# COMP6248-Reproducability-Challenge/selfsupervised-denoising

Hardware: AMD Instinct MI355X
Metric: training patches/sec (64x64 gauss25 SSDN) (higher is better)
Workload: dtype f16

## Files before the change

### include/ssdn_hip.h

```cpp
#ifndef SSDN_HIP_H
#define SSDN_HIP_H

#include <stdint.h>

#ifdef __cplusplus
extern "C" {
#endif
#if defined(__GNUC__) || defined(__clang__)
#pragma GCC visibility push(default)
#endif

#define SSDN_ABI_VERSION 19
#define SSDN_MAX_TAPS 9

typedef struct ssdn_view {
    void* p;
    int32_t cs;
    int32_t co;
} ssdn_view;

enum ssdn_op_type {
    SSDN_OP_PACK_INPUT = 1,
    SSDN_OP_CONV = 2,
    SSDN_OP_POOL_FWD = 3,
// ... 362 lines not shown
int ssdn_run_ops(const ssdn_op* ops, int n, void* stream);

int ssdn_stream_order(void* first, void* then);

int ssdn_conv_lds_bytes(const ssdn_conv_args* a);
int ssdn_wgrad_lds_bytes(const ssdn_wgrad_args* a);
int ssdn_wgrad_mega_ok(const ssdn_wgrad_args* a);
int ssdn_wgrad_variant(const ssdn_wgrad_args* a, int32_t* out9);

int ssdn_struct_size(int op_type);
int ssdn_abi_version(void);
const char* ssdn_last_error(void);
int ssdn_device_cus(void);

#define SSDN_PROF_CONV_MT3 0
#define SSDN_PROF_CONV_MT2 1
#define SSDN_PROF_CONV_MT1 2
#define SSDN_PROF_WGRAD 3
#define SSDN_PROF_GEMM 4
#define SSDN_PROF_CDMA_MT3 5
#define SSDN_PROF_CDMA_MT21 6
#define SSDN_PROF_WGRAD_SIDE 7
#define SSDN_PROF_KINDS 8
int ssdn_profile_enable(int kind, int max_launches);
int ssdn_profile_set_stride(int kind, int stride);
int ssdn_profile_read(int kind, double* total_ms, long long* launches, double* flops, double* bytes);

int ssdn_conv_set_mode(int mode);
int ssdn_conv_fuses_pool(const ssdn_conv_args* a);
int ssdn_conv_fuses_upsum(const ssdn_conv_args* a);
int ssdn_conv_fuses_unrot(const ssdn_conv_args* a);
int ssdn_conv_fuses_urot(const ssdn_conv_args* a);
int ssdn_conv_signs(const ssdn_conv_args* a);

int ssdn_chain_len(const ssdn_op* ops, int n);
int ssdn_conv_set_chain(int on);

int ssdn_wgrad_mergeable(const ssdn_wgrad_args* a);

#define SSDN_PLAN_REPACK 0
#define SSDN_PLAN_FORWARD 1
#define SSDN_PLAN_BACKWARD 2
#define SSDN_PLAN_OPTIMISER 3
#define SSDN_PLAN_PHASES 4
typedef struct ssdn_plan ssdn_plan;
int ssdn_plan_load(const void* blob, int64_t nbytes, ssdn_plan** out);
void ssdn_plan_destroy(ssdn_plan* plan);
int64_t ssdn_plan_arena_bytes(const ssdn_plan* plan);
const char* ssdn_plan_meta(const ssdn_plan* plan);
int ssdn_plan_bind(ssdn_plan* plan, void* arena);
int ssdn_plan_tensor(const ssdn_plan* plan, const char* name, void** ptr, int64_t* bytes);
int ssdn_plan_run(ssdn_plan* plan, int phase, void* stream);
int ssdn_plan_set_lr(ssdn_plan* plan, float lr, int step, float gscale);
int ssdn_net_forward(ssdn_plan* plan, void* stream);
int ssdn_train_step(ssdn_plan* plan, float lr, int step, void* stream);

void ssdn_debug_set_trace(void* device_buffer);
void* ssdn_debug_get_trace(void);

int ssdn_probe_mfma(const void* a_frag, const void* b_frag, float* d_out, void* stream);
int ssdn_probe_tr16(const void* lds_image, int image_bytes, const int32_t* lane_addr, void* out, void* stream);

#if defined(__GNUC__) || defined(__clang__)
#pragma GCC visibility pop
#endif
#ifdef __cplusplus
// ... 4 lines not shown
```

### selfsupervised-denoising_amd/csrc/api.hip

```cpp
#include "common.h"
#include <cstdarg>
#include <cstdio>
#include <cstdlib>

static thread_local char g_err[512] = "";
thread_local hipEvent_t g_ssdn_stop_event = nullptr;
thread_local bool g_ssdn_stop_used = false;
thread_local hipEvent_t g_ssdn_prof_start = nullptr, g_ssdn_prof_stop = nullptr;
thread_local bool g_ssdn_prof_used = false;

int ssdn_set_error(const char* fmt, ...) {
    va_list ap;
    va_start(ap, fmt);
    vsnprintf(g_err, sizeof(g_err), fmt, ap);
    va_end(ap);
    return -1;
}

#include <vector>
struct ProfSlot {
    bool on = false;
    std::vector<hipEvent_t> ev;
    size_t used = 0;
    double flops = 0.0, bytes = 0.0;
// ... 107 lines not shown
    if (stride < 1) return ssdn_set_error("profile: stride must be >= 1");
    g_prof[kind].stride = stride;
    return 0;
}

int ssdn_profile_read(int kind, double* total_ms, long long* launches, double* flops, double* bytes) {
    if (kind < 0 || kind >= SSDN_PROF_KINDS) return ssdn_set_error("profile: bad kernel kind %d", kind);
    ProfSlot& p = g_prof[kind];
    double ms = 0.0;
    for (size_t i = 0; i + 1 < p.used; i += 2) {
        if (hipEventSynchronize(p.ev[i + 1]) != hipSuccess) return ssdn_set_error("profile: hipEventSynchronize failed");
        float t = 0.f;
        if (hipEventElapsedTime(&t, p.ev[i], p.ev[i + 1]) != hipSuccess) return ssdn_set_error("profile: hipEventElapsedTime failed");
        ms += t;
    }
    *total_ms = ms;
    *launches = (long long)(p.used / 2);
    *flops = p.flops;
    *bytes = p.bytes;
    p.used = 0;
    p.flops = p.bytes = 0.0;
    return 0;
}

int ssdn_conv_lds_bytes(const ssdn_conv_args* a) { return conv_lds_bytes(a); }
int ssdn_wgrad_lds_bytes(const ssdn_wgrad_args* a) { return wgrad_lds_bytes(a); }
int ssdn_wgrad_mergeable(const ssdn_wgrad_args* a) { return a && wgrad_mergeable(a) ? 1 : 0; }
int ssdn_wgrad_mega_ok(const ssdn_wgrad_args* a) { return wgrad_mega_ok(a); }
int ssdn_conv_fuses_pool(const ssdn_conv_args* a) { return a && conv_fuses_pool(a) ? 1 : 0; }
int ssdn_conv_fuses_upsum(const ssdn_conv_args* a) { return a && conv_fuses_upsum(a) ? 1 : 0; }
int ssdn_conv_fuses_unrot(const ssdn_conv_args* a) { return a && conv_fuses_unrot(a) ? 1 : 0; }
int ssdn_conv_fuses_urot(const ssdn_conv_args* a) { return a && conv_fuses_urot(a) ? 1 : 0; }
int ssdn_conv_signs(const ssdn_conv_args* a) { return a && conv_signs(a) ? 1 : 0; }

#define SSDN_NEVENTS 256
#define SSDN_NLANES 4
#define SSDN_MAX_DEVICES 16
struct LaneSet {
    hipStream_t side[SSDN_NLANES] = {nullptr, nullptr, nullptr, nullptr};
    hipEvent_t ev[SSDN_NEVENTS];
    int ev_next = 0;
    bool ready = false;
};
static LaneSet g_lanesets[SSDN_MAX_DEVICES];
static LaneSet* lanes_get() {
    int dev = 0;
    if (hipGetDevice(&dev) != hipSuccess || dev < 0 || dev >= SSDN_MAX_DEVICES) { ssdn_set_error("lanes: bad current device"); return nullptr; }
    LaneSet& L = g_lanesets[dev];
    if (L.ready) return &L;
    for (int l = 1; l < SSDN_NLANES; ++l)
        if (hipStreamCreateWithFlags(&L.side[l], hipStreamNonBlocking) != hipSuccess) { ssdn_set_error("lanes: hipStreamCreate failed"); return nullptr; }
    for (int i = 0; i < SSDN_NEVENTS; ++i)
        if (hipEventCreateWithFlags(&L.ev[i], hipEventDisableTiming) != hipSuccess) { ssdn_set_error("lanes: hipEventCreate failed"); return nullptr; }
    L.ready = true;
    return &L;
}
static const unsigned g_lane_deps[SSDN_NLANES] = {0u, 1u << 0, (1u << 0) | (1u << 1) | (1u << 3), 1u << 0};

int ssdn_stream_order(void* first, void* then) {
    LaneSet* LS = lanes_get();
    if (!LS) return -1;
    hipEvent_t e = LS->ev[LS->ev_next++ % SSDN_NEVENTS];
    SSDN_CHECK_HIP(hipEventRecord(e, (hipStream_t)first));
    SSDN_CHECK_HIP(hipStreamWaitEvent((hipStream_t)then, e, 0));
    return 0;
}
// ... 265 lines not shown
```

### selfsupervised-denoising_amd/csrc/common.h

```cpp
#pragma once
#include <hip/hip_runtime.h>
#include <hip/hip_ext.h>
#include <stdint.h>
#include "../../include/ssdn_hip.h"
#include <cstdlib>

#if defined(SSDN_TUNING)
static inline const char* ssdn_tuning_env(const char* name) { return std::getenv(name); }
#else
static inline const char* ssdn_tuning_env(const char*) { return nullptr; }
#endif

typedef _Float16 h16;
typedef _Float16 half8 __attribute__((ext_vector_type(8)));
typedef _Float16 half4 __attribute__((ext_vector_type(4)));
typedef _Float16 half2v __attribute__((ext_vector_type(2)));
typedef __bf16 bf16x8 __attribute__((ext_vector_type(8)));
typedef unsigned short u16x8 __attribute__((ext_vector_type(8)));
typedef unsigned short u16x4 __attribute__((ext_vector_type(4)));
typedef float f32x16 __attribute__((ext_vector_type(16)));
typedef float f32x4 __attribute__((ext_vector_type(4)));

#define LRELU_SLOPE 0.1f

// ... 105 lines not shown
int launch_spatial_mean(const ssdn_spatial_mean_args* a, hipStream_t s);
int launch_mse(const ssdn_mse_args* a, int masked, hipStream_t s);
int launch_head_vjp(const ssdn_head_vjp_args* a, hipStream_t s);
int launch_head_vjp_impulse(const ssdn_head_vjp_args* a, hipStream_t s);
int launch_head_posterior(const ssdn_head_posterior_args* a, hipStream_t s);
int launch_ssim(const ssdn_ssim_args* a, hipStream_t s);
int launch_calibration(const ssdn_calibration_args* a, hipStream_t s);
int launch_mse_vjp(const ssdn_mse_vjp_args* a, hipStream_t s);
int launch_adam(const ssdn_adam_args* a, hipStream_t s);
#define ADAM_PACK_MAX 24
int adam_pack_fusable(const ssdn_adam_args* a, const ssdn_wpack_args* const* items, int n);
int launch_adam_pack(const ssdn_adam_args* a, const ssdn_wpack_args* const* items, int n, hipStream_t s);
int tail_fused_ok(const ssdn_wreduce_args* const* wr, int nw, const ssdn_adam_args* a, const ssdn_wpack_args* const* wp, int np);
int launch_tail_fused(const ssdn_wreduce_args* const* wr, int nw, const ssdn_adam_args* a, const ssdn_wpack_args* const* wp, int np, hipStream_t s);
int launch_metrics(const ssdn_metrics_args* a, hipStream_t s);
int launch_accum(const ssdn_accum_args* a, hipStream_t s);
int launch_noise(const ssdn_noise_args* a, hipStream_t s);
int launch_input_grad(const ssdn_input_grad_args* a, hipStream_t s);
int conv_lds_bytes(const ssdn_conv_args* a);
int conv_validate(const ssdn_conv_args* a);
int chain_len(const ssdn_op* ops, int n, bool any_lane);
int launch_chain(const ssdn_op* ops, int n, bool any_lane, hipStream_t s);
bool chain_merging_on();
bool conv_dma_eligible(const ssdn_conv_args* a, bool any_size);
int conv_dma_lds_bytes(int mt);
bool conv_signs(const ssdn_conv_args* a);
bool gemm_dma_signs(const ssdn_conv_args* a);
bool conv_dma_signs(const ssdn_conv_args* a);
bool conv_fuses_urot(const ssdn_conv_args* a);
bool conv_fuses_unrot(const ssdn_conv_args* a);
bool conv_fuses_upsum(const ssdn_conv_args* a);
bool conv_fuses_pool(const ssdn_conv_args* a);
int launch_conv_dma(const ssdn_conv_args* a, hipStream_t s);
bool conv_thin_eligible(const ssdn_conv_args* a);
bool conv_thin_fuses_pack(const ssdn_pack_input_args* pk, const ssdn_conv_args* a);
int launch_conv_thin(const ssdn_conv_args* a, const ssdn_pack_input_args* pk, hipStream_t s);
bool conv_pack_fusable(const ssdn_pack_input_args* pk, const ssdn_conv_args* a);
bool gradpack_dgrad_fusable(const ssdn_grad_pack_args* gp, const ssdn_conv_args* a);
int launch_gradpack_dgrad(const ssdn_grad_pack_args* gp, const ssdn_conv_args* a, hipStream_t s);
bool conv_gradpack_fusable(const ssdn_grad_pack_args* gp, const ssdn_conv_args* a);
bool gemm_dma_eligible(const ssdn_conv_args* a);
int gemm_dma_lds_bytes(const ssdn_conv_args* a);
int launch_gemm_dma(const ssdn_conv_args* a, hipStream_t s);
bool gemm_dma_fuses_next(const ssdn_conv_args* a, const ssdn_conv_args* b);
int launch_gemm_dma_with_next(const ssdn_conv_args* a, const ssdn_conv_args* b, hipStream_t s);
bool conv_pair_fusable(const ssdn_conv_args* a, const ssdn_conv_args* b);
extern "C" int ssdn_device_cus(void);
int wgrad_lds_bytes(const ssdn_wgrad_args* a);
```

### selfsupervised-denoising_amd/csrc/conv_mfma.hip

```cpp
#include "common.h"
#ifdef SSDN_TUNING
#define CV_ABL(xx, bit) (((xx).ablate & (bit)) != 0)
#define CV_TUNING 1
#else
#define CV_ABL(xx, bit) false
#define CV_TUNING 0
#endif
#include <cstdlib>


struct ConvGeom {
    int TW, TH, TN, HH, HW, padT, padB, padL, padR;
    int PSTR, WSTR, NP;
    int tiles_x, tiles_y, groups_n;
};

static __host__ __device__ inline ConvGeom conv_geom(int ltw, int lth, int ltn, int ntaps, const int* dy, const int* dx,
                                                     int N, int H, int W, int kc) {
    ConvGeom g;
    g.TW = 1 << ltw; g.TH = 1 << lth; g.TN = 1 << ltn;
    int mny = 0, mxy = 0, mnx = 0, mxx = 0;
    for (int t = 0; t < ntaps; ++t) {
        mny = dy[t] < mny ? dy[t] : mny; mxy = dy[t] > mxy ? dy[t] : mxy;
        mnx = dx[t] < mnx ? dx[t] : mnx; mxx = dx[t] > mxx ? dx[t] : mxx;
// ... 631 lines not shown
                    }
                    if (has_mask) {
                        v0 *= lrelu_grad(f16_lo(mb[w]));
                        v1 *= lrelu_grad(f16_hi(mb[w]));
                    }
                    o[w] = BF ? pack_bf16x2(v0, v1) : pack_f16x2(v0, v1);
                }
            }
            __builtin_amdgcn_raw_buffer_store_b128(o, rd[u], go[u], 0, 0);
        }
    }
    stamp();
}

static bool conv_uses_mt1(const ssdn_conv_args* a, const ConvGeom& g) {
    static int mt1_tiles = -1;
    if (mt1_tiles < 0) {
        const char* e = ssdn_tuning_env("SSDN_CONV_MT1_TILES");
        mt1_tiles = e ? atoi(e) : ssdn_device_cus();
        if (mt1_tiles <= 0) mt1_tiles = 256;
    }
    return !a->dst32 && g.tiles_x * g.tiles_y * g.groups_n <= mt1_tiles && a->Mpad >= 64;
}

static int g_conv_mode = [] { const char* e = ssdn_tuning_env("SSDN_CONV_DMA"); return e ? atoi(e) : 1; }();
extern "C" int ssdn_conv_set_mode(int mode) {
    if (mode < 0 || mode > 2) return ssdn_set_error("conv mode must be 0, 1 or 2");
    g_conv_mode = mode;
    return 0;
}
static bool conv_use_dma(const ssdn_conv_args* a) { return g_conv_mode > 0 && !a->pool.p && conv_dma_eligible(a, g_conv_mode == 2); }
static bool conv_use_gemm(const ssdn_conv_args* a) { return g_conv_mode > 0 && gemm_dma_eligible(a); }
static bool conv_use_thin(const ssdn_conv_args* a) { return g_conv_mode > 0 && conv_thin_eligible(a); }
bool conv_gradpack_fusable(const ssdn_grad_pack_args* gp, const ssdn_conv_args* a) {
    return !conv_validate(a) && !conv_use_gemm(a) && !conv_use_thin(a) && !conv_use_dma(a) && gradpack_dgrad_fusable(gp, a);
}
bool conv_pair_fusable(const ssdn_conv_args* a, const ssdn_conv_args* b) {
    return !conv_validate(a) && !conv_validate(b) && conv_use_gemm(a) && gemm_dma_fuses_next(a, b);
}
bool conv_pack_fusable(const ssdn_pack_input_args* pk, const ssdn_conv_args* a) {
    return !conv_validate(a) && !conv_use_gemm(a) && conv_use_thin(a) && conv_thin_fuses_pack(pk, a);
}

int conv_validate(const ssdn_conv_args* a) {
    if (a->ntaps < 1 || a->ntaps > SSDN_MAX_TAPS) return ssdn_set_error("conv: ntaps out of range");
    if (a->ltw + a->lth + a->ltn > 9 || a->ltw < 0 || a->lth < 0 || a->ltn < 0) return ssdn_set_error("conv: tile must have <= 512 pixels");
    if (a->Ktot != a->c0 + a->c1 || (a->Ktot & 15)) return ssdn_set_error("conv: Ktot must equal c0+c1 and be a multiple of 16");
    if ((a->c0 & 7) || (a->c1 & 7)) return ssdn_set_error("conv: source channel counts must be multiples of 8");
    if (a->kc < 16 || (a->kc & 15) || a->Ktot % a->kc || (a->kc > 64 && a->kc != 96)) return ssdn_set_error("conv: kc must be 16, 32, 48, 64 or 96 and divide Ktot");
    if ((a->Mpad & 31) || a->M > a->Mpad) return ssdn_set_error("conv: Mpad must be a multiple of 32 and >= M");
    if (!a->dst32 && ((a->M & 7) || (a->dst.co & 7) || (a->dst.cs & 7))) return ssdn_set_error("conv: 16-bit output needs M, dst.co, dst.cs %% 8 == 0");
    if (a->add.p && ((a->add.co & 7) || (a->add.cs & 7))) return ssdn_set_error("conv: add view must be 16-byte aligned");
    if (a->mask.p && ((a->mask.co & 7) || (a->mask.cs & 7))) return ssdn_set_error("conv: mask view must be 16-byte aligned");
    if (a->up0 && ((a->H | a->W) & 1)) return ssdn_set_error("conv: upsampled source needs even H, W");
    if (a->c1 > 0 && !a->src1.p) return ssdn_set_error("conv: src1 missing");
    if (a->bf16 && a->dst32) return ssdn_set_error("conv: fp32 output is only implemented for the fp16 (forward) role");
    int csmax = a->src0.cs > a->src1.cs ? a->src0.cs : a->src1.cs;
    if ((long long)a->N * a->H * a->W * csmax >= (1ll << 31)) return ssdn_set_error("conv: tensor too large for 32-bit element offsets");
    return 0;
}

static size_t conv_lds(const ssdn_conv_args* a, const ConvGeom& g, int mt) {
    size_t main_b = (conv_async(*a, a->kc) ? 2 * (size_t)g.NP * a->kc * 2 : (size_t)g.NP * g.PSTR) + 2 * (size_t)mt * 32 * g.WSTR;
    if (conv_allw(*a, g, mt, a->kc) && !conv_async(*a, a->kc)) main_b = (size_t)g.NP * g.PSTR + 9 * (size_t)32 * g.WSTR;
    size_t epi_b = a->dst32 ? 0 : (size_t)(g.TN * g.TH * g.TW) * (mt * 64 + 16) + mt * 32 * 4;
    return main_b > epi_b ? main_b : epi_b;
}

int conv_lds_bytes(const ssdn_conv_args* a) {
    if (conv_validate(a)) return -1;
    if (conv_use_gemm(a)) return gemm_dma_lds_bytes(a);
    if (conv_use_thin(a)) return 32 * 1024;
    if (conv_use_dma(a)) return conv_dma_lds_bytes(a->Mpad >= 96 ? 3 : a->Mpad / 32);
    ConvGeom g = conv_geom(a->ltw, a->lth, a->ltn, a->ntaps, a->dy, a->dx, a->N, a->H, a->W, a->kc);
    int mt = a->Mpad / 32;
    if (mt > 3) mt = 3;
    if (conv_uses_mt1(a, g)) mt = 1;
    else if (a->kc == 96) { ssdn_set_error("conv: kc = 96 is only built for layers that run as 32-channel blocks (<= 1 tile per CU)"); return -1; }
    return (int)conv_lds(a, g, mt);
}

static bool conv_flat_ok(const ssdn_conv_args* a, const ConvGeom& g, int ks, int threads) {
    static const bool no_flat = ssdn_tuning_env("SSDN_CONV_NO_FLAT") != nullptr;
    const int m_last = a->M - (a->Mpad - 32);
    return !no_flat && threads == 256 && ks <= 4 && g.TW == a->W && g.TH == a->H && g.TN * g.TH * g.TW == 256 && a->N % g.TN == 0 &&
           (m_last == 32 || m_last == 16 || m_last == 8) && (!a->up0 || !((a->H | a->W) & 1));
}

template <int MT, bool BF, int KS, int CONV_THREADS>
static int conv_launch_mt(const ssdn_conv_args* a, const ConvGeom& g, ConvAux x, int nblk_y, hipStream_t s) {
    size_t lds = conv_lds(a, g, MT);
    if (lds > 160 * 1024) return ssdn_set_error("conv: tiling needs %zu B of LDS (> 160 KiB)", lds);
    static bool attr_set_dev[SSDN_MAX_DEVICES_ATTR] = {};
    bool& attr_set = attr_set_dev[ssdn_current_device_slot()];
    if (!attr_set) {
        SSDN_CHECK_HIP(hipFuncSetAttribute((const void*)k_conv<MT, BF, KS, CONV_THREADS>, hipFuncAttributeMaxDynamicSharedMemorySize, 160 * 1024));
        attr_set = true;
    }
    int grid = g.tiles_x * g.tiles_y * g.groups_n;
    int m_real = a->M - x.m_base;
    m_real = m_real < 0 ? 0 : (m_real > nblk_y * MT * 32 ? nblk_y * MT * 32 : m_real);
    double px = (double)a->N * a->H * a->W;
    const int kreal = a->kreal > 0 ? a->kreal : a->Ktot;
    double flops = 2.0 * px * m_real * kreal * a->ntaps;
    double bytes = px * (a->c0 * 2.0 / (a->up0 ? 4.0 : 1.0) + a->c1 * 2.0) + px * m_real * (a->dst32 ? 4.0 : 2.0);
    prof_begin(3 - MT, s);
// ... 45 lines not shown
bool conv_signs(const ssdn_conv_args* a) {
    if (!(a->sign_out || a->mask_sign || a->upsum_mask_sign) || conv_validate(a)) return false;
    if (conv_use_gemm(a)) return !a->upsum_mask_sign && gemm_dma_signs(a);
    if (conv_use_thin(a)) return a->sign_out && !a->mask_sign && !a->upsum_mask_sign;
    return conv_use_dma(a) && conv_dma_signs(a);
}
bool conv_fuses_urot(const ssdn_conv_args* a) {
    return a->urot.p && !conv_validate(a) && !conv_use_gemm(a) && !conv_use_thin(a) && conv_use_dma(a);
}
bool conv_fuses_unrot(const ssdn_conv_args* a) {
    ssdn_conv_args q = *a;
    if (!q.unrot.p) { q.unrot = q.dst; q.unrot_mask = q.dst; }
    return !conv_validate(&q) && conv_use_gemm(&q);
}
bool conv_fuses_upsum(const ssdn_conv_args* a) {
    if (conv_validate(a) || !a->bf16 || a->dst32 || a->mask.p || a->add.p || (a->H & 1) || (a->W & 1)) return false;
    if ((a->upsum_c & 7) || a->upsum_c > a->M || a->upsum_c <= 0) return false;
    if (conv_use_gemm(a)) return false;
    if (conv_use_dma(a)) return a->upsum_c % 96 == 0;
    return conv_flat_path(a);
}

int launch_conv(const ssdn_conv_args* a, hipStream_t s) {
    int rc = conv_validate(a);
    if (rc) return rc;
    if ((a->sign_out || a->mask_sign || a->upsum_mask_sign) && !conv_signs(a)) return ssdn_set_error("conv: sign bytes requested for a launch that cannot write / read them (ssdn_conv_signs)");
    if (a->urot.p && !conv_fuses_urot(a)) return ssdn_set_error("conv: fused UNROT_FWD requested for a launch that cannot fuse it (ssdn_conv_fuses_urot)");
    if (a->unrot.p && !conv_fuses_unrot(a)) return ssdn_set_error("conv: fused UNROT_BWD requested for a launch that cannot fuse it (ssdn_conv_fuses_unrot)");
    if (a->upsum.p && !conv_fuses_upsum(a)) return ssdn_set_error("conv: fused upsum requested for a launch that cannot fuse it (ssdn_conv_fuses_upsum)");
    if (a->pool.p && !conv_fuses_pool(a)) return ssdn_set_error("conv: fused max-pool requested for a launch that cannot fuse it (ssdn_conv_fuses_pool)");
    if (conv_use_gemm(a)) return launch_gemm_dma(a, s);
    if (conv_use_thin(a)) return launch_conv_thin(a, nullptr, s);
    if (conv_use_dma(a)) return launch_conv_dma(a, s);
    ConvGeom g = conv_geom(a->ltw, a->lth, a->ltn, a->ntaps, a->dy, a->dx, a->N, a->H, a->W, a->kc);
    ConvAux x;
    x.mg_hw = magic_of(g.HW);
    x.mg_hh = magic_of(g.HH);
    x.mg_ntaps = magic_of(a->ntaps);
    x.m_base = 0;
    {
        static const int env_ablate = [] { const char* e = ssdn_tuning_env("SSDN_CONV_ABLATE"); return e ? atoi(e) : 0; }();
        static const int env_desync = [] { const char* e = ssdn_tuning_env("SSDN_CONV_DESYNC"); return e ? atoi(e) : 0; }();
        x.ablate = env_ablate;
        x.trace = g_conv_trace;
        x.desync = env_desync;
    }
    int full = a->Mpad / 96, rem = (a->Mpad % 96) / 32;
    const bool bf = a->bf16 != 0;
    if (conv_uses_mt1(a, g)) {
        rc = bf ? conv_launch_ks<1, true>(a, g, x, a->Mpad / 32, s) : conv_launch_ks<1, false>(a, g, x, a->Mpad / 32, s);
        if (rc) return rc;
        SSDN_CHECK_HIP(hipGetLastError());
        return 0;
    }
    if (full) {
        rc = bf ? conv_launch_ks<3, true>(a, g, x, full, s) : conv_launch_ks<3, false>(a, g, x, full, s);
        if (rc) return rc;
    }
    x.m_base = full * 96;
    if (rem == 2) rc = bf ? conv_launch_ks<2, true>(a, g, x, 1, s) : conv_launch_ks<2, false>(a, g, x, 1, s);
    else if (rem == 1) rc = bf ? conv_launch_ks<1, true>(a, g, x, 1, s) : conv_launch_ks<1, false>(a, g, x, 1, s);
    if (rc) return rc;
    SSDN_CHECK_HIP(hipGetLastError());
    return 0;
}
```

### selfsupervised-denoising_amd/ssdn/hip/lib.py

```python
from __future__ import annotations

import ctypes as C
import os

_HERE = os.path.dirname(os.path.abspath(__file__))
LIB_PATH = os.environ.get("SSDN_HIP_LIB") or os.path.join(_HERE, "libssdn_hip.so")
MAX_TAPS = 9

OP = dict(pack_input=1, conv=2, pool_fwd=3, pool_bwd=4, upsum_bwd=5, unrot_fwd=6, unrot_bwd=7, wgrad=8, wreduce=9,
          wpack=10, grad_pack=11, head_ssdn=12, head_final=13, spatial_mean=14, mse=15, mask_mse=16, adam=17,
          metrics=18, zero=19, event_record=20, noise=21, input_grad=22, head_vjp=23,
          mse_vjp=24, accum=25, head_posterior=26, ssim=27, calibration=28)

i32, f32, vp = C.c_int32, C.c_float, C.c_void_p


class View(C.Structure):
    _fields_ = [("p", vp), ("cs", i32), ("co", i32)]


class OpRec(C.Structure):
    _fields_ = [("type", i32), ("lane", i32), ("args", vp)]


# ... 126 lines not shown
SSIM_WIN, SSIM_TILE_H, SSIM_TILE_W = 11, 16, 32


def ssim_scratch_bytes(B: int, Cn: int, H: int, W: int) -> int:
    tiles = lambda n, t: (n - (SSIM_WIN - 1) + t - 1) // t
    return 8 * B * Cn * tiles(H, SSIM_TILE_H) * tiles(W, SSIM_TILE_W)


class CalibrationArgs(C.Structure):
    _fields_ = [("mean", vp), ("cov", vp), ("ref", vp), ("ext", vp), ("B", i32), ("C", i32), ("H", i32), ("W", i32), ("stats", vp),
                ("hist", vp), ("zmap", vp), ("scratch", vp), ("scratch_bytes", C.c_int64)]


CALIB_BLOCK, CALIB_NSTATS, CALIB_HIST_BINS = 256, 12, 34


def calib_scratch_bytes(B: int, Cn: int, H: int, W: int) -> int:
    return 8 * CALIB_NSTATS * B * ((H * W + CALIB_BLOCK - 1) // CALIB_BLOCK)


ARG_TYPES = dict(pack_input=PackInputArgs, conv=ConvArgs, pool_fwd=PoolArgs, pool_bwd=PoolArgs, upsum_bwd=UpsumArgs,
                 unrot_fwd=UnrotArgs, unrot_bwd=UnrotArgs, wgrad=WgradArgs, wreduce=WreduceArgs, wpack=WpackArgs,
                 grad_pack=GradPackArgs, head_ssdn=HeadArgs, head_final=HeadFinalArgs, spatial_mean=SpatialMeanArgs,
                 mse=MseArgs, mask_mse=MseArgs, adam=AdamArgs, metrics=MetricsArgs, zero=ZeroArgs, event_record=EventArgs, noise=NoiseArgs,
                 input_grad=InputGradArgs, head_vjp=HeadVjpArgs, mse_vjp=MseVjpArgs, accum=AccumArgs,
                 head_posterior=HeadPosteriorArgs, ssim=SsimArgs, calibration=CalibrationArgs)

ABI_VERSION = 19

SYMBOLS = ["ssdn_run_ops", "ssdn_stream_order", "ssdn_conv_lds_bytes", "ssdn_wgrad_lds_bytes", "ssdn_abi_version", "ssdn_last_error",
           "ssdn_device_cus", "ssdn_probe_mfma", "ssdn_probe_tr16", "ssdn_struct_size", "ssdn_profile_enable",
           "ssdn_profile_read", "ssdn_profile_set_stride", "ssdn_debug_set_trace", "ssdn_debug_get_trace", "ssdn_conv_set_mode",
           "ssdn_wgrad_mergeable", "ssdn_conv_fuses_pool", "ssdn_conv_fuses_upsum", "ssdn_conv_fuses_unrot", "ssdn_conv_fuses_urot", "ssdn_conv_signs", "ssdn_chain_len",
           "ssdn_conv_set_chain", "ssdn_wgrad_mega_ok", "ssdn_wgrad_variant",
           "ssdn_plan_load", "ssdn_plan_destroy", "ssdn_plan_arena_bytes", "ssdn_plan_meta", "ssdn_plan_bind", "ssdn_plan_tensor", "ssdn_plan_run",
           "ssdn_plan_set_lr", "ssdn_net_forward", "ssdn_train_step"]
PLAN_PHASES = dict(repack=0, forward=1, backward=2, optimiser=3)
PROF = dict(conv_mt3=0, conv_mt2=1, conv_mt1=2, wgrad=3, gemm=4, cdma_mt3=5, cdma_mt21=6, wgrad_side=7)

def pointer_fields(st, base: int = 0):
    out = []
    for name, ty in st._fields_:
        off = base + getattr(st, name).offset
        if ty is vp:
            out.append(off)
        elif isinstance(ty, type) and issubclass(ty, C.Structure):
            out += pointer_fields(ty, off)
    return out


_lib = None


class SsdnHipError(RuntimeError):
    pass


def load() -> C.CDLL:
    global _lib
    if _lib is not None:
        return _lib
    if not os.path.exists(LIB_PATH):
        raise SsdnHipError("libssdn_hip.so not found at %s -- build it with `python -c 'import __graft_entry__ as g; g.build()'` "
                           "(the ssdn hot path has no CPU fallback)" % LIB_PATH)
    lib = C.CDLL(LIB_PATH)
    lib.ssdn_run_ops.argtypes = [C.POINTER(OpRec), C.c_int, vp]
    lib.ssdn_run_ops.restype = C.c_int
# ... 3 lines not shown
    lib.ssdn_conv_lds_bytes.argtypes = [C.POINTER(ConvArgs)]
    lib.ssdn_conv_lds_bytes.restype = C.c_int
    lib.ssdn_wgrad_lds_bytes.argtypes = [C.POINTER(WgradArgs)]
    lib.ssdn_wgrad_lds_bytes.restype = C.c_int
    lib.ssdn_abi_version.restype = C.c_int
    lib.ssdn_last_error.restype = C.c_char_p
    lib.ssdn_device_cus.restype = C.c_int
    lib.ssdn_probe_mfma.argtypes = [vp, vp, vp, vp]
    lib.ssdn_probe_mfma.restype = C.c_int
    lib.ssdn_probe_tr16.argtypes = [vp, C.c_int, vp, vp, vp]
    lib.ssdn_probe_tr16.restype = C.c_int
    lib.ssdn_profile_enable.argtypes = [C.c_int, C.c_int]
    lib.ssdn_profile_enable.restype = C.c_int
    lib.ssdn_profile_set_stride.argtypes = [C.c_int, C.c_int]
    lib.ssdn_profile_set_stride.restype = C.c_int
    lib.ssdn_profile_read.argtypes = [C.c_int, C.POINTER(C.c_double), C.POINTER(C.c_longlong), C.POINTER(C.c_double), C.POINTER(C.c_double)]
    lib.ssdn_profile_read.restype = C.c_int
    lib.ssdn_conv_set_mode.argtypes = [C.c_int]
    lib.ssdn_conv_set_mode.restype = C.c_int
    lib.ssdn_conv_set_chain.argtypes = [C.c_int]
    lib.ssdn_conv_set_chain.restype = C.c_int
    lib.ssdn_chain_len.argtypes = [C.c_void_p, C.c_int]
    lib.ssdn_chain_len.restype = C.c_int
    lib.ssdn_conv_fuses_unrot.argtypes = [C.c_void_p]
    lib.ssdn_conv_fuses_unrot.restype = C.c_int
    lib.ssdn_conv_fuses_urot.argtypes = [C.c_void_p]
    lib.ssdn_conv_fuses_urot.restype = C.c_int
    lib.ssdn_conv_signs.argtypes = [C.c_void_p]
    lib.ssdn_conv_signs.restype = C.c_int
    lib.ssdn_conv_fuses_upsum.argtypes = [C.c_void_p]
    lib.ssdn_conv_fuses_upsum.restype = C.c_int
    lib.ssdn_conv_fuses_pool.argtypes = [C.c_void_p]
    lib.ssdn_conv_fuses_pool.restype = C.c_int
    lib.ssdn_wgrad_mergeable.argtypes = [C.c_void_p]
    lib.ssdn_wgrad_mergeable.restype = C.c_int
    lib.ssdn_wgrad_mega_ok.argtypes = [C.c_void_p]
    lib.ssdn_wgrad_mega_ok.restype = C.c_int
    lib.ssdn_wgrad_variant.argtypes = [C.c_void_p, C.POINTER(C.c_int32)]
    lib.ssdn_wgrad_variant.restype = C.c_int
    lib.ssdn_struct_size.argtypes = [C.c_int]
    lib.ssdn_struct_size.restype = C.c_int
    lib.ssdn_plan_load.argtypes = [C.c_void_p, C.c_int64, C.POINTER(C.c_void_p)]
    lib.ssdn_plan_load.restype = C.c_int
    lib.ssdn_plan_destroy.argtypes = [C.c_void_p]
    lib.ssdn_plan_destroy.restype = None
    lib.ssdn_plan_arena_bytes.argtypes = [C.c_void_p]
    lib.ssdn_plan_arena_bytes.restype = C.c_int64
    lib.ssdn_plan_meta.argtypes = [C.c_void_p]
    lib.ssdn_plan_meta.restype = C.c_char_p
    lib.ssdn_plan_bind.argtypes = [C.c_void_p, C.c_void_p]
    lib.ssdn_plan_bind.restype = C.c_int
    lib.ssdn_plan_tensor.argtypes = [C.c_void_p, C.c_char_p, C.POINTER(C.c_void_p), C.POINTER(C.c_int64)]
    lib.ssdn_plan_tensor.restype = C.c_int
    lib.ssdn_plan_run.argtypes = [C.c_void_p, C.c_int, C.c_void_p]
    lib.ssdn_plan_run.restype = C.c_int
    lib.ssdn_plan_set_lr.argtypes = [C.c_void_p, C.c_float, C.c_int, C.c_float]
    lib.ssdn_plan_set_lr.restype = C.c_int
    lib.ssdn_net_forward.argtypes = [C.c_void_p, C.c_void_p]
    lib.ssdn_net_forward.restype = C.c_int
    lib.ssdn_train_step.argtypes = [C.c_void_p, C.c_float, C.c_int, C.c_void_p]
    lib.ssdn_train_step.restype = C.c_int
    if lib.ssdn_abi_version() != ABI_VERSION:
        raise SsdnHipError("libssdn_hip.so ABI version mismatch")
    if os.environ.get("SSDN_CHAIN_MODE"):
        lib.ssdn_conv_set_chain(int(os.environ["SSDN_CHAIN_MODE"]))
    _lib = lib
    return lib


def check(rc: int):
    if rc != 0:
        raise SsdnHipError(load().ssdn_last_error().decode())
```

Before: 22050.

## Add specialized 16x16 conv kernel with LDS-DMA weight ring for bf16 roles

Adds a dedicated MFMA conv kernel for 16x16 spatial, 9-tap layers with 96/144 channels. Each block stages a half-image halo tile into LDS once and streams weight slices through a multi-slot LDS ring using buffer loads that write directly to LDS. It also fuses bias, activation, residual add, mask and the bf16 upsample-sum epilogue. By default it is enabled only for bf16 (backward-gradient) convolutions that would otherwise take the generic flat path. This targets the generic path's overhead at small resolutions, at the cost of large LDS use and low occupancy.

```diff
diff --git a/include/ssdn_hip.h b/include/ssdn_hip.h
--- a/include/ssdn_hip.h
+++ b/include/ssdn_hip.h
@@ -418,6 +418,8 @@
 int ssdn_conv_fuses_unrot(const ssdn_conv_args* a);
 int ssdn_conv_fuses_urot(const ssdn_conv_args* a);
 int ssdn_conv_signs(const ssdn_conv_args* a);
+int ssdn_conv16_eligible(const ssdn_conv_args* a);
+int ssdn_conv_set_conv16(int roles);
 
 int ssdn_chain_len(const ssdn_op* ops, int n);
 int ssdn_conv_set_chain(int on);
diff --git a/selfsupervised-denoising_amd/csrc/api.hip b/selfsupervised-denoising_amd/csrc/api.hip
--- a/selfsupervised-denoising_amd/csrc/api.hip
+++ b/selfsupervised-denoising_amd/csrc/api.hip
@@ -163,6 +163,7 @@
 int ssdn_conv_fuses_unrot(const ssdn_conv_args* a) { return a && conv_fuses_unrot(a) ? 1 : 0; }
 int ssdn_conv_fuses_urot(const ssdn_conv_args* a) { return a && conv_fuses_urot(a) ? 1 : 0; }
 int ssdn_conv_signs(const ssdn_conv_args* a) { return a && conv_signs(a) ? 1 : 0; }
+int ssdn_conv16_eligible(const ssdn_conv_args* a) { return a && conv_use_conv16(a) ? 1 : 0; }
 
 #define SSDN_NEVENTS 256
 #define SSDN_NLANES 4
diff --git a/selfsupervised-denoising_amd/csrc/common.h b/selfsupervised-denoising_amd/csrc/common.h
--- a/selfsupervised-denoising_amd/csrc/common.h
+++ b/selfsupervised-denoising_amd/csrc/common.h
@@ -161,6 +161,10 @@
 bool conv_fuses_upsum(const ssdn_conv_args* a);
 bool conv_fuses_pool(const ssdn_conv_args* a);
 int launch_conv_dma(const ssdn_conv_args* a, hipStream_t s);
+bool conv16_shape_ok(const ssdn_conv_args* a);
+bool conv_use_conv16(const ssdn_conv_args* a);
+int conv16_lds_bytes(const ssdn_conv_args* a);
+int launch_conv16(const ssdn_conv_args* a, hipStream_t s);
 bool conv_thin_eligible(const ssdn_conv_args* a);
 bool conv_thin_fuses_pack(const ssdn_pack_input_args* pk, const ssdn_conv_args* a);
 int launch_conv_thin(const ssdn_conv_args* a, const ssdn_pack_input_args* pk, hipStream_t s);
diff --git a/selfsupervised-denoising_amd/csrc/conv16.hip b/selfsupervised-denoising_amd/csrc/conv16.hip
--- /dev/null
+++ b/selfsupervised-denoising_amd/csrc/conv16.hip
@@ -0,0 +1,335 @@
+#include "common.h"
+
+#define C16_THREADS 256
+#define C16_HW 18
+#define C16_HH 10
+#define C16_NP (C16_HW * C16_HH)
+#define C16_WROW 7
+
+struct C16Aux {
+    int padT, padL;
+    int pa, pb;
+    unsigned mg_pa, mg_pb;
+    int rega, tile_bytes;
+};
+
+static __device__ __forceinline__ unsigned c16_fdiv(unsigned v, unsigned magic) { return magic ? __umulhi(v, magic) : v; }
+static inline unsigned c16_magic(unsigned d) { return d <= 1 ? 0u : (unsigned)((0x100000000ull + d - 1) / d); }
+
+static __device__ __forceinline__ void c16_dma(unsigned lds_dst, int voff, u32x4_t rs) {
+    asm volatile("s_nop 4\n\ts_mov_b32 m0, %0\n\ts_nop 0\n\tbuffer_load_dwordx4 %1, %2, 0 offen lds" :: "s"(lds_dst), "v"(voff), "s"(rs) : "memory");
+}
+template <int N>
+static __device__ __forceinline__ void c16_wait_barrier() {
+    asm volatile("s_waitcnt vmcnt(%0)\n\ts_waitcnt lgkmcnt(0)\n\ts_barrier" :: "n"(N) : "memory");
+}
+
+template <bool BF>
+static __device__ __forceinline__ f32x16 c16_mma(half8 av, half8 bv, f32x16 c) {
+    if constexpr (BF)
+        return __builtin_amdgcn_mfma_f32_32x32x16_bf16(__builtin_bit_cast(bf16x8, av), __builtin_bit_cast(bf16x8, bv), c, 0, 0, 0);
+    else
+        return __builtin_amdgcn_mfma_f32_32x32x16_f16(av, bv, c, 0, 0, 0);
+}
+
+#ifndef C16_RING_F
+#define C16_RING_F 8
+#endif
+#ifndef C16_RING_B3
+#define C16_RING_B3 3
+#endif
+#ifndef C16_RING_B5
+#define C16_RING_B5 2
+#endif
+#ifndef C16_OCC_B3
+#define C16_OCC_B3 2
+#endif
+#ifndef C16_OCC_B5
+#define C16_OCC_B5 2
+#endif
+static constexpr __host__ __device__ int c16_ring(int mt, bool bf) { return !bf ? C16_RING_F : (mt == 3 ? C16_RING_B3 : C16_RING_B5); }
+static constexpr __host__ __device__ int c16_occ(int mt, bool bf) { return !bf ? 1 : (mt == 3 ? C16_OCC_B3 : C16_OCC_B5); }
+
+template <int MT>
+struct C16Frag {
+    half8 b[3];
+    half8 a[3][MT];
+};
+
+template <int MT, bool BF>
+__global__ __launch_bounds__(C16_THREADS, c16_occ(MT, BF)) void k_conv16(ssdn_conv_args a, C16Aux x) {
+    constexpr int R = c16_ring(MT, BF);
+    static_assert(R >= 2 && R <= 10, "ring depth");
+    constexpr int WROWS = MT * 32;
+    constexpr int IPW = (WROWS * C16_WROW + 255) / 256;
+    constexpr int SLOT = IPW * 4 * 1024;
+    constexpr int WSTR = C16_WROW * 16;
+    constexpr int M = MT == 3 ? 96 : 144;
+    constexpr int CPP = M / 8;
+    extern __shared__ __attribute__((aligned(16))) char smem[];
+    const int tid = threadIdx.x, lane = tid & 63, l31 = lane & 31, kh = lane >> 5;
+    const int wave = __builtin_amdgcn_readfirstlane(tid >> 6);
+    const int img = (int)((blockIdx.x >> 4) * 8 + (blockIdx.x & 7)), half = (int)(blockIdx.x >> 3) & 1;
+    if (img >= a.N) return;
+    const bool cm = a.wc != nullptr;
+    const unsigned pf = __builtin_amdgcn_raw_buffer_load_b32(
+        __builtin_amdgcn_make_buffer_rsrc(const_cast<void*>(cm ? a.wc : a.w), 0, 9 * a.Mpad * a.Ktot * 2, SSDN_BUFFER_RSRC_FLAGS),
+        (int)(((blockIdx.x >> 3) * C16_THREADS + tid) << 7), 0, 0);
+
+    const unsigned lds0 = (unsigned)(size_t)smem;
+    const int y0 = half * 8;
+    const int nchunks = a.Ktot / 48;
+
+    auto stage_region = [&](const ssdn_view& v, int c, int up, int P, unsigned mgP, unsigned ldsb) __attribute__((always_inline)) {
+        const int hs = up ? 8 : 16;
+        const unsigned long long bp = (unsigned long long)((const h16*)v.p + ((long long)img * hs * hs * v.cs + v.co));
+        const u32x4_t rs = {(unsigned)bp, (unsigned)(bp >> 32) & 0xffffu, (unsigned)(((hs * hs - 1) * v.cs + c) * 2), SSDN_BUFFER_RSRC_FLAGS};
+        const int total = C16_NP * P, npieces = (total + 63) >> 6;
+        for (int i = wave; i < npieces; i += 4) {
+            const int p = i * 64 + lane;
+            const int hp = (int)c16_fdiv((unsigned)p, mgP), cc = p - hp * P;
+            const int hy = hp / C16_HW, hx = hp - hy * C16_HW;
+            const int y = y0 - x.padT + hy, xx = hx - x.padL;
+            const bool ok = p < total && cc < P - 1 && (unsigned)y < 16u && (unsigned)xx < 16u;
+            const int pix = up ? ((y >> 1) * 8 + (xx >> 1)) : (y * 16 + xx);
+            c16_dma(ldsb + (unsigned)i * 1024u, ok ? (pix * v.cs + cc * 8) * 2 : (int)0x80000000, rs);
+        }
+    };
+    if (x.pa) stage_region(a.src0, a.c0, a.up0, x.pa, x.mg_pa, lds0);
+    if (x.pb) stage_region(a.src1, a.c1, 0, x.pb, x.mg_pb, lds0 + (unsigned)x.rega);
+
+    int woff[IPW];
+#pragma unroll
+    for (int j = 0; j < IPW; ++j) {
+        const int p = (j * 4 + wave) * 64 + lane;
+        const int r = p / C16_WROW, cc = p - r * C16_WROW;
+        const int src = cm ? r * 96 + ((cc ^ ((r >> 3) & 1)) << 4) : (r * a.Ktot + cc * 8) * 2;
+        woff[j] = (cc < C16_WROW - 1 && r < WROWS) ? src : (int)0x80000000;
+    }
+    const unsigned ring = lds0 + (unsigned)x.tile_bytes;
+    const unsigned wrec = cm ? (unsigned)(WROWS * 96) : (unsigned)(((WROWS - 1) * a.Ktot + 48) * 2);
+    auto issue_slice = [&](int ch, int t, int slot) __attribute__((always_inline)) {
+        const long long el = cm ? ((long long)(t * nchunks + ch) * a.Mpad * 48) : ((long long)t * a.Mpad * a.Ktot + ch * 48);
+        const unsigned long long bp = (unsigned long long)((const h16*)(cm ? a.wc : a.w) + el);
+        const u32x4_t rs = {(unsigned)bp, (unsigned)(bp >> 32) & 0xffffu, wrec, SSDN_BUFFER_RSRC_FLAGS};
+#pragma unroll
+        for (int j = 0; j < IPW; ++j) c16_dma(ring + (unsigned)(slot * SLOT + (j * 4 + wave) * 1024), woff[j], rs);
+    };
+#pragma unroll
+    for (int s = 0; s < R; ++s) issue_slice(s / 9, s % 9, s);
+
+    const int q = wave * 32 + l31;
+    const int hpl = ((q >> 4) + x.padT) * C16_HW + (q & 15) + x.padL;
+    const int bA = hpl * x.pa * 16 + kh * 16;
+    const int bB = x.rega + hpl * x.pb * 16 + kh * 16;
+    const int aoff = x.tile_bytes + l31 * WSTR + kh * 16;
+    auto load_frag = [&](C16Frag<MT>& f, int ch, int dyx, int slot) __attribute__((always_inline)) {
+        const bool in_a = ch * 48 < a.c0;
+        const char* bp = smem + (in_a ? bA : bB) + (in_a ? ch * 48 : ch * 48 - a.c0) * 2 + dyx * ((in_a ? x.pa : x.pb) * 16);
+        const char* ap = smem + aoff + slot * SLOT;
+#pragma unroll
+        for (int ks = 0; ks < 3; ++ks) {
+            f.b[ks] = *reinterpret_cast<const half8*>(bp + ks * 32);
+#pragma unroll
+            for (int mt = 0; mt < MT; ++mt) f.a[ks][mt] = *reinterpret_cast<const half8*>(ap + mt * 32 * WSTR + ks * 32);
+        }
+    };
+
+    f32x16 acc[MT];
+#pragma unroll
+    for (int mt = 0; mt < MT; ++mt)
+#pragma unroll
+        for (int r = 0; r < 16; ++r) acc[mt][r] = 0.f;
+
+    C16Frag<MT> cur, nxt;
+    c16_wait_barrier<(R - 1) * IPW>();
+    load_frag(cur, 0, a.dy[0] * C16_HW + a.dx[0], 0);
+    for (int ch = 0; ch < nchunks; ++ch) {
+        const bool last = ch + 1 == nchunks;
+#pragma unroll
+        for (int t = 0; t < 9; ++t) {
+            const int s = ch * 9 + t;
+            constexpr int full = (R - 2) * IPW;
+            const int tail = IPW * (R - 2 < 7 - t ? R - 2 : (7 - t > 0 ? 7 - t : 0));
+            if (!last) c16_wait_barrier<full>();
+            else switch (tail) {
+                case 0: c16_wait_barrier<0>(); break;
+                case IPW: c16_wait_barrier<IPW>(); break;
+                case 2 * IPW: c16_wait_barrier<2 * IPW>(); break;
+                case 3 * IPW: c16_wait_barrier<3 * IPW>(); break;
+                case 4 * IPW: c16_wait_barrier<4 * IPW>(); break;
+                case 5 * IPW: c16_wait_barrier<5 * IPW>(); break;
+                case 6 * IPW: c16_wait_barrier<6 * IPW>(); break;
+                default: c16_wait_barrier<0>(); break;
+            }
+            const int t2 = (t + R) % 9, ch2 = ch + (t + R) / 9;
+            if (ch2 < nchunks) issue_slice(ch2, t2, s % R);
+            const int t1 = (t + 1) % 9;
+            if (t < 8 || !last) load_frag(nxt, ch + (t + 1) / 9, a.dy[t1] * C16_HW + a.dx[t1], (s + 1) % R);
+#pragma unroll
+            for (int ks = 0; ks < 3; ++ks)
+#pragma unroll
+                for (int mt = 0; mt < MT; ++mt) acc[mt] = c16_mma<BF>(cur.a[ks][mt], cur.b[ks], acc[mt]);
+            cur = nxt;
+        }
+    }
+    c16_wait_barrier<0>();
+    asm volatile("" :: "v"(pf));
+
+    constexpr int OSTR = MT * 64 + 16;
+    char* ot = smem;
+    float* bl = reinterpret_cast<float*>(smem + (size_t)128 * OSTR);
+    if (tid < WROWS) bl[tid] = (a.bias && tid < a.M) ? a.bias[tid] : 0.f;
+    __syncthreads();
+#pragma unroll
+    for (int mt = 0; mt < MT; ++mt) {
+#pragma unroll
+        for (int gq = 0; gq < 4; ++gq) {
+            const int ml = mt * 32 + gq * 8 + kh * 4;
+            const f32x4 bb = *reinterpret_cast<const f32x4*>(bl + ml);
+            float v[4];
+#pragma unroll
+            for (int j = 0; j < 4; ++j) {
+                v[j] = acc[mt][gq * 4 + j] + bb[j];
+                if (a.act) v[j] = lrelu(v[j]);
+            }
+            u32x2_t o;
+            o[0] = BF ? pack_bf16x2(v[0], v[1]) : pack_f16x2(v[0], v[1]);
+            o[1] = BF ? pack_bf16x2(v[2], v[3]) : pack_f16x2(v[2], v[3]);
+            *reinterpret_cast<u32x2_t*>(ot + q * OSTR + ml * 2) = o;
+        }
+    }
+    __syncthreads();
+    const long long pixb = (long long)img * 256 + half * 128;
+    const bool has_mask = a.mask.p != nullptr, has_add = a.add.p != nullptr;
+    constexpr int NU = 128 * CPP / C16_THREADS;
+    static_assert(128 * CPP % C16_THREADS == 0, "pieces of the half tile must divide over the threads");
+    half8 mk[NU], ad[NU];
+#pragma unroll
+    for (int u = 0; u < NU; ++u) {
+        const int e = tid + u * C16_THREADS;
+        const int pq = e / CPP, c = e - pq * CPP;
+        mk[u] = zero_h8(); ad[u] = zero_h8();
+        if (has_mask) mk[u] = ld_h8((const h16*)a.mask.p + ((pixb + pq) * a.mask.cs + a.mask.co + c * 8));
+        if (has_add) ad[u] = ld_h8((const h16*)a.add.p + ((pixb + pq) * a.add.cs + a.add.co + c * 8));
+    }
+#pragma unroll
+    for (int u = 0; u < NU; ++u) {
+        const int e = tid + u * C16_THREADS;
+        const int pq = e / CPP, c = e - pq * CPP;
+        if (a.upsum.p && c * 8 < a.upsum_c) continue;
+        u32x4_t o = *reinterpret_cast<const u32x4_t*>(ot + pq * OSTR + c * 16);
+        if (has_add || has_mask) {
+            const u32x4_t ab = __builtin_bit_cast(u32x4_t, ad[u]), mb = __builtin_bit_cast(u32x4_t, mk[u]);
+#pragma unroll
+            for (int w = 0; w < 4; ++w) {
+                float v0, v1;
+                if constexpr (BF) {
+                    v0 = bf_lo(o[w]) + (has_add ? bf_lo(ab[w]) : 0.f);
+                    v1 = bf_hi(o[w]) + (has_add ? bf_hi(ab[w]) : 0.f);
+                } else {
+                    v0 = f16_lo(o[w]) + (has_add ? f16_lo(ab[w]) : 0.f);
+                    v1 = f16_hi(o[w]) + (has_add ? f16_hi(ab[w]) : 0.f);
+                }
+                if (has_mask) {
+                    v0 *= lrelu_grad(f16_lo(mb[w]));
+                    v1 *= lrelu_grad(f16_hi(mb[w]));
+                }
+                o[w] = BF ? pack_bf16x2(v0, v1) : pack_f16x2(v0, v1);
+            }
+        }
+        *reinterpret_cast<u32x4_t*>((h16*)a.dst.p + ((pixb + pq) * a.dst.cs + a.dst.co + c * 8)) = o;
+    }
+    if constexpr (BF) {
+        if (a.upsum.p) {
+            const int ucp = a.upsum_c >> 3;
+            for (int e = tid; e < 32 * ucp; e += C16_THREADS) {
+                const int pp_l = e / ucp, c = e - pp_l * ucp;
+                const int pi = pp_l >> 3, pj = pp_l & 7;
+                const long long pp = ((long long)img * 8 + half * 4 + pi) * 8 + pj;
+                const u32x4_t um = *reinterpret_cast<const u32x4_t*>((const h16*)a.upsum_mask.p + (pp * a.upsum_mask.cs + a.upsum_mask.co + c * 8));
+                float sum[8] = {0.f, 0.f, 0.f, 0.f, 0.f, 0.f, 0.f, 0.f};
+#pragma unroll
+                for (int q4 = 0; q4 < 4; ++q4) {
+                    const u32x4_t o = *reinterpret_cast<const u32x4_t*>(ot + ((2 * pi + (q4 >> 1)) * 16 + 2 * pj + (q4 & 1)) * OSTR + c * 16);
+#pragma unroll
+                    for (int k = 0; k < 4; ++k) { sum[2 * k] += bf_lo(o[k]); sum[2 * k + 1] += bf_hi(o[k]); }
+                }
+                u32x4_t r;
+#pragma unroll
+                for (int k = 0; k < 4; ++k)
+                    r[k] = pack_bf16x2(sum[2 * k] * lrelu_grad(f16_lo(um[k])), sum[2 * k + 1] * lrelu_grad(f16_hi(um[k])));
+                *reinterpret_cast<u32x4_t*>((h16*)a.upsum.p + (pp * a.upsum.cs + a.upsum.co + c * 8)) = r;
+            }
+        }
+    }
+}
+
+static C16Aux c16_aux(const ssdn_conv_args* a) {
+    C16Aux x;
+    int mny = 0, mnx = 0;
+    for (int t = 0; t < a->ntaps; ++t) {
+        mny = a->dy[t] < mny ? a->dy[t] : mny;
+        mnx = a->dx[t] < mnx ? a->dx[t] : mnx;
+    }
+    x.padT = -mny; x.padL = -mnx;
+    x.pa = a->c0 > 0 ? a->c0 / 8 + 1 : 0;
+    x.pb = a->c1 > 0 ? a->c1 / 8 + 1 : 0;
+    x.mg_pa = c16_magic((unsigned)x.pa); x.mg_pb = c16_magic((unsigned)x.pb);
+    x.rega = (C16_NP * x.pa * 16 + 1023) & ~1023;
+    x.tile_bytes = x.rega + ((C16_NP * x.pb * 16 + 1023) & ~1023);
+    return x;
+}
+
+static int c16_lds(const ssdn_conv_args* a) {
+    const int mt = a->Mpad / 32;
+    const int slot = ((mt * 32 * C16_WROW + 255) / 256) * 4 * 1024;
+    const int main_b = c16_aux(a).tile_bytes + c16_ring(mt, a->bf16 != 0) * slot;
+    const int epi_b = 128 * (mt * 64 + 16) + mt * 32 * 4;
+    return main_b > epi_b ? main_b : epi_b;
+}
+
+bool conv16_shape_ok(const ssdn_conv_args* a) {
+    if (a->ntaps != 9 || a->H != 16 || a->W != 16 || a->ltw != 4 || a->lth != 4 || a->ltn != 0 || a->kc != 48) return false;
+    if ((a->Ktot != 96 && a->Ktot != 144) || a->c0 % 48 || a->c1 % 48 || a->c0 + a->c1 != a->Ktot) return false;
+    if (a->up0 && a->c0 == 0) return false;
+    if (!((a->Mpad == 96 && a->M == 96) || (a->Mpad == 160 && a->M == 144 && a->bf16))) return false;
+    if (a->dst32 || a->pool.p || a->urot.p || a->unrot.p || a->urot_smask || a->unrot_smask || a->sign_out || a->mask_sign || a->upsum_mask_sign) return false;
+    if (a->upsum.p && (!a->bf16 || (a->upsum_c & 7) || a->upsum_c <= 0 || a->upsum_c > a->M)) return false;
+    int mny = 0, mxy = 0, mnx = 0, mxx = 0;
+    for (int t = 0; t < 9; ++t) {
+        mny = a->dy[t] < mny ? a->dy[t] : mny; mxy = a->dy[t] > mxy ? a->dy[t] : mxy;
+        mnx = a->dx[t] < mnx ? a->dx[t] : mnx; mxx = a->dx[t] > mxx ? a->dx[t] : mxx;
+    }
+    return mxy - mny == C16_HH - 8 && mxx - mnx == C16_HW - 16;
+}
+
+int conv16_lds_bytes(const ssdn_conv_args* a) { return c16_lds(a); }
+
+template <int MT, bool BF>
+static int c16_launch(const ssdn_conv_args* a, hipStream_t s) {
+    const size_t lds = (size_t)c16_lds(a);
+    if (lds > 160 * 1024) return ssdn_set_error("conv16: needs %zu B of LDS (> 160 KiB)", lds);
+    static bool attr_set_dev[SSDN_MAX_DEVICES_ATTR] = {};
+    bool& attr_set = attr_set_dev[ssdn_current_device_slot()];
+    if (!attr_set) {
+        SSDN_CHECK_HIP(hipFuncSetAttribute((const void*)k_conv16<MT, BF>, hipFuncAttributeMaxDynamicSharedMemorySize, 160 * 1024));
+        attr_set = true;
+    }
+    const double px = (double)a->N * a->H * a->W;
+    const int kreal = a->kreal > 0 ? a->kreal : a->Ktot;
+    const double flops = 2.0 * px * a->M * kreal * a->ntaps;
+    const double bytes = px * (a->c0 * 2.0 / (a->up0 ? 4.0 : 1.0) + a->c1 * 2.0) + px * a->M * 2.0;
+    const int grid = ((2 * a->N + 15) / 16) * 16;
+    prof_begin(SSDN_PROF_CONV_MT1, s);
+    SSDN_LAUNCH((k_conv16<MT, BF>), dim3(grid), dim3(C16_THREADS), lds, s, *a, c16_aux(a));
+    prof_end(SSDN_PROF_CONV_MT1, s, flops, bytes);
+    SSDN_CHECK_HIP(hipGetLastError());
+    return 0;
+}
+
+int launch_conv16(const ssdn_conv_args* a, hipStream_t s) {
+    if (!conv16_shape_ok(a)) return ssdn_set_error("conv16: not a launch of its shape class");
+    if (a->Mpad == 160) return c16_launch<5, true>(a, s);
+    return a->bf16 ? c16_launch<3, true>(a, s) : c16_launch<3, false>(a, s);
+}
diff --git a/selfsupervised-denoising_amd/csrc/conv_mfma.hip b/selfsupervised-denoising_amd/csrc/conv_mfma.hip
--- a/selfsupervised-denoising_amd/csrc/conv_mfma.hip
+++ b/selfsupervised-denoising_amd/csrc/conv_mfma.hip
@@ -687,6 +687,18 @@
 static bool conv_use_dma(const ssdn_conv_args* a) { return g_conv_mode > 0 && !a->pool.p && conv_dma_eligible(a, g_conv_mode == 2); }
 static bool conv_use_gemm(const ssdn_conv_args* a) { return g_conv_mode > 0 && gemm_dma_eligible(a); }
 static bool conv_use_thin(const ssdn_conv_args* a) { return g_conv_mode > 0 && conv_thin_eligible(a); }
+static bool conv_flat_path(const ssdn_conv_args* a);
+#define CONV16_DEFAULT_ROLES 2
+static int g_conv16_roles = CONV16_DEFAULT_ROLES;
+extern "C" int ssdn_conv_set_conv16(int roles) {
+    if (roles < -1 || roles > 3) return ssdn_set_error("conv16 roles must be -1 .. 3");
+    g_conv16_roles = roles < 0 ? CONV16_DEFAULT_ROLES : roles;
+    return 0;
+}
+bool conv_use_conv16(const ssdn_conv_args* a) {
+    return g_conv_mode > 0 && (g_conv16_roles & (a->bf16 ? 2 : 1)) && !conv_validate(a) && conv16_shape_ok(a) && !conv_use_gemm(a) &&
+           !conv_use_thin(a) && !conv_use_dma(a) && conv_flat_path(a);
+}
 bool conv_gradpack_fusable(const ssdn_grad_pack_args* gp, const ssdn_conv_args* a) {
     return !conv_validate(a) && !conv_use_gemm(a) && !conv_use_thin(a) && !conv_use_dma(a) && gradpack_dgrad_fusable(gp, a);
 }
@@ -727,6 +739,7 @@
     if (conv_use_gemm(a)) return gemm_dma_lds_bytes(a);
     if (conv_use_thin(a)) return 32 * 1024;
     if (conv_use_dma(a)) return conv_dma_lds_bytes(a->Mpad >= 96 ? 3 : a->Mpad / 32);
+    if (conv_use_conv16(a)) return conv16_lds_bytes(a);
     ConvGeom g = conv_geom(a->ltw, a->lth, a->ltn, a->ntaps, a->dy, a->dx, a->N, a->H, a->W, a->kc);
     int mt = a->Mpad / 32;
     if (mt > 3) mt = 3;
@@ -838,6 +851,7 @@
     if (conv_use_gemm(a)) return launch_gemm_dma(a, s);
     if (conv_use_thin(a)) return launch_conv_thin(a, nullptr, s);
     if (conv_use_dma(a)) return launch_conv_dma(a, s);
+    if (conv_use_conv16(a)) return launch_conv16(a, s);
     ConvGeom g = conv_geom(a->ltw, a->lth, a->ltn, a->ntaps, a->dy, a->dx, a->N, a->H, a->W, a->kc);
     ConvAux x;
     x.mg_hw = magic_of(g.HW);
diff --git a/selfsupervised-denoising_amd/ssdn/hip/lib.py b/selfsupervised-denoising_amd/ssdn/hip/lib.py
--- a/selfsupervised-denoising_amd/ssdn/hip/lib.py
+++ b/selfsupervised-denoising_amd/ssdn/hip/lib.py
@@ -182,7 +182,7 @@
            "ssdn_device_cus", "ssdn_probe_mfma", "ssdn_probe_tr16", "ssdn_struct_size", "ssdn_profile_enable",
            "ssdn_profile_read", "ssdn_profile_set_stride", "ssdn_debug_set_trace", "ssdn_debug_get_trace", "ssdn_conv_set_mode",
            "ssdn_wgrad_mergeable", "ssdn_conv_fuses_pool", "ssdn_conv_fuses_upsum", "ssdn_conv_fuses_unrot", "ssdn_conv_fuses_urot", "ssdn_conv_signs", "ssdn_chain_len",
-           "ssdn_conv_set_chain", "ssdn_wgrad_mega_ok", "ssdn_wgrad_variant",
+           "ssdn_conv_set_chain", "ssdn_wgrad_mega_ok", "ssdn_wgrad_variant", "ssdn_conv16_eligible", "ssdn_conv_set_conv16",
            "ssdn_plan_load", "ssdn_plan_destroy", "ssdn_plan_arena_bytes", "ssdn_plan_meta", "ssdn_plan_bind", "ssdn_plan_tensor", "ssdn_plan_run",
            "ssdn_plan_set_lr", "ssdn_net_forward", "ssdn_train_step"]
 PLAN_PHASES = dict(repack=0, forward=1, backward=2, optimiser=3)
@@ -252,6 +252,11 @@
     lib.ssdn_conv_fuses_upsum.restype = C.c_int
     lib.ssdn_conv_fuses_pool.argtypes = [C.c_void_p]
     lib.ssdn_conv_fuses_pool.restype = C.c_int
+    if hasattr(lib, "ssdn_conv16_eligible"):
+        lib.ssdn_conv16_eligible.argtypes = [C.c_void_p]
+        lib.ssdn_conv16_eligible.restype = C.c_int
+        lib.ssdn_conv_set_conv16.argtypes = [C.c_int]
+        lib.ssdn_conv_set_conv16.restype = C.c_int
     lib.ssdn_wgrad_mergeable.argtypes = [C.c_void_p]
     lib.ssdn_wgrad_mergeable.restype = C.c_int
     lib.ssdn_wgrad_mega_ok.argtypes = [C.c_void_p]
@@ -284,6 +289,8 @@
         raise SsdnHipError("libssdn_hip.so ABI version mismatch")
     if os.environ.get("SSDN_CHAIN_MODE"):
         lib.ssdn_conv_set_chain(int(os.environ["SSDN_CHAIN_MODE"]))
+    if os.environ.get("SSDN_CONV16_ROLES") and hasattr(lib, "ssdn_conv_set_conv16"):
+        lib.ssdn_conv_set_conv16(int(os.environ["SSDN_CONV16_ROLES"]))
     _lib = lib
     return lib
 
```

New measurement: 22330 (median of 6 runs). +1.3%, better.
